# HazyResearch/hyena-dna

Measured on NVIDIA H100. Metric: nucleotides/sec through HyenaOperator fwd+bwd at L=1M d=256, higher is better.
Workload: dtype f32

## Files before the change

hyena-dna_b200/csrc/filter_tc.cuh:

```cuda
#pragma once
#include "fft_passes.cuh"
#include "filter_mlp.cuh"
#include "tc_prims.cuh"

namespace hy {
namespace tc {

constexpr int kTileM = 128;
constexpr uint32_t kSBO = 2048, kLBO = 128;
constexpr int kImgW64 = 64 * 64;
constexpr int kImgW128 = 128 * 64;

__host__ __device__ constexpr uint32_t op_off(int r, int k) {
  return (uint32_t)((r >> 3) * 2048 + (k >> 2) * 128 + (r & 7) * 16 + (k & 3) * 4);
}

constexpr uint32_t kOffAhi = 0, kOffAlo = 32768, kOffW1hi = 65536, kOffW1lo = 81920, kOffW2hi = 98304,
                   kOffW2lo = 114688, kOffW3hi = 131072, kOffW3lo = 163840, kOffMisc = 196608;
constexpr uint32_t kMiscFloats = 64 * 16 + 4 * 64;
constexpr size_t kSmemBytes = kOffMisc + kMiscFloats * 4 + 16;

__host__ __device__ constexpr size_t wimg_floats(int D) { return 4 * (size_t)kImgW64 + (size_t)((D + 127) / 128) * 2 * kImgW128; }

__device__ __noinline__ float sin_ni(float x) { return sinf(x); }
__device__ __noinline__ float cos_ni(float x) { return cosf(x); }

__device__ __forceinline__ void sincos_core(float x, float& sn, float& cs, int& q) {
  const float fq = rintf(x * 0.636619772367581343f);
  q = (int)fq;
  float r = fmaf(fq, -1.5707963705062866f, x);
  r = fmaf(fq, 4.371138828673793e-08f, r);
  r = fmaf(fq, 1.7763568394002505e-15f, r);
  const float s = r * r;
  float ps = fmaf(-1.95152959e-4f, s, 8.33216087e-3f);
  ps = fmaf(ps, s, -1.66666546e-1f);
  sn = fmaf(ps, s * r, r);
  float pc = fmaf(2.44331571e-5f, s, -1.38873163e-3f);
  pc = fmaf(pc, s, 4.16666457e-2f);
  pc = fmaf(pc, s, -0.5f);
  cs = fmaf(pc, s, 1.0f);
}
__device__ __forceinline__ float sin_acc(float x) {
  if (fabsf(x) > 30000.f) return sin_ni(x);
  float sn, cs; int q;
  sincos_core(x, sn, cs, q);
  const float v = (q & 1) ? cs : sn;
  return (q & 2) ? -v : v;
}
__device__ __forceinline__ float cos_acc(float x) {
  if (fabsf(x) > 30000.f) return cos_ni(x);
  float sn, cs; int q;
  sincos_core(x, sn, cs, q);
  const float v = (q & 1) ? sn : cs;
  return ((q + 1) & 2) ? -v : v;
}

struct Frag {
  int r0, t, rh, ch;
  __device__ Frag(int tid) {
    const int warp = tid >> 5, lane = tid & 31, wg = warp >> 2;
    rh = wg & 1; ch = wg >> 1; t = lane & 3;
    r0 = 64 * rh + 16 * (warp & 3) + (lane >> 2);
  }
  __device__ int row(int i) const { return r0 + ((i & 2) ? 8 : 0); }
  __device__ int col(int i, int n_half) const { return ch * n_half + 8 * (i >> 2) + 2 * t + (i & 1); }
};

template <int R>
__device__ __forceinline__ void layer_ss(float (&m)[R], float (&c)[R], uint32_t a_hi, uint32_t a_lo, uint32_t b_hi,
                                         uint32_t b_lo, uint32_t acc0) {
  wgmma_fence();
  fence_regs(m); fence_regs(c);
#pragma unroll
  for (int ks = 0; ks < 8; ++ks)
    wgmma_ss(m, make_desc_ls(a_hi + ks * 2 * kLBO, kLBO, kSBO), make_desc_ls(b_hi + ks * 2 * kLBO, kLBO, kSBO), (acc0 | ks) ? 1u : 0u);
#pragma unroll
  for (int ks = 0; ks < 8; ++ks) {
    wgmma_ss(c, make_desc_ls(a_lo + ks * 2 * kLBO, kLBO, kSBO), make_desc_ls(b_hi + ks * 2 * kLBO, kLBO, kSBO), (acc0 | ks) ? 1u : 0u);
    wgmma_ss(c, make_desc_ls(a_hi + ks * 2 * kLBO, kLBO, kSBO), make_desc_ls(b_lo + ks * 2 * kLBO, kLBO, kSBO), 1u);
  }
  wgmma_commit();
}
template <int R>
__device__ __forceinline__ void layer_wait(float (&m)[R], float (&c)[R]) {
  wgmma_wait<0>();
  fence_regs(m); fence_regs(c);
}

__device__ __forceinline__ void store_pair_split(unsigned char* smem, int r, int k, float x0, float x1) {
  float2 hi, lo;
  split_tf32(x0, hi.x, lo.x);
  split_tf32(x1, hi.y, lo.y);
  const uint32_t off = op_off(r, k);
  *reinterpret_cast<float2*>(smem + kOffAhi + off) = hi;
  *reinterpret_cast<float2*>(smem + kOffAlo + off) = lo;
}
__device__ __forceinline__ void store_frag16(unsigned char* smem, const Frag& f, const float (&a)[16]) {
#pragma unroll
  for (int i = 0; i < 16; i += 2) store_pair_split(smem, f.row(i), f.col(i, 32), a[i], a[i + 1]);
}
__device__ __forceinline__ uint32_t a_rows(uint32_t img, const Frag& f) { return img + (uint32_t)f.rh * 8u * kSBO; }

__global__ void filter_tc_prep_kernel(const float* __restrict__ W1, const float* __restrict__ W2,
                                      const float* __restrict__ W3, int D, float* __restrict__ wimg) {
  const int nh = (D + 127) / 128;
  const int total = 2 * kImgW64 + nh * kImgW128;
  for (int i = blockIdx.x * blockDim.x + threadIdx.x; i < total; i += gridDim.x * blockDim.x) {
    float x;
    float* hi_img;
    float* lo_img;
    int r, k;
    if (i < 2 * kImgW64) {
      const int w = i / kImgW64, e = i % kImgW64;
      r = e / 64; k = e % 64;
      x = (w == 0 ? W1 : W2)[r * 64 + k];
      hi_img = wimg + w * 2 * kImgW64;
      lo_img = hi_img + kImgW64;
    } else {
      const int j = i - 2 * kImgW64, h = j / kImgW128, e = j % kImgW128;
      r = e / 64; k = e % 64;
      const int c = h * 128 + r;
      x = (c < D) ? W3[(size_t)c * 64 + k] : 0.f;
      hi_img = wimg + 4 * kImgW64 + (size_t)h * 2 * kImgW128;
      lo_img = hi_img + kImgW128;
    }
    float hi, lo;
    split_tf32(x, hi, lo);
    hi_img[op_off(r, k) / 4] = hi;
    lo_img[op_off(r, k) / 4] = lo;
  }
}

constexpr int kThreads = 512;

__global__ void __launch_bounds__(kThreads, 1)
filter_tc_fwd_kernel(const FilterParams P, const float* __restrict__ wimg, float* __restrict__ kout, int ntiles) {
  extern __shared__ __align__(1024) unsigned char smem[];
  float* misc = reinterpret_cast<float*>(smem + kOffMisc);
  float* W0s = misc;
  float* b0s = misc + 64 * 16;
  float* b1s = b0s + 64;
  float* b2s = b1s + 64;
  float* frs = b2s + 64;
  const int tid = threadIdx.x;
  const Frag f(tid);
  const uint32_t sbase = smem_u32(smem);
  const int nh = (P.D + 127) / 128;

  for (int i = tid; i < 4 * kImgW64 / 4; i += kThreads)
    cp_async16(smem + kOffW1hi + 16 * i, wimg + 4 * i, true);
  for (int i = tid; i < 64 * 16; i += kThreads) {
    const int r = i / 16, e = i % 16;
    W0s[i] = (e < P.E) ? __ldg(P.W0 + r * P.E + e) : 0.f;
  }
  if (tid < 64) {
    b0s[tid] = __ldg(P.b0 + tid); b1s[tid] = __ldg(P.b1 + tid); b2s[tid] = __ldg(P.b2 + tid);
    frs[tid] = __ldg(P.freq + tid);
  }
  cp_async_wait_all();
  __syncthreads();
  const uint32_t a_hi = a_rows(sbase + kOffAhi, f), a_lo = a_rows(sbase + kOffAlo, f);

  for (int tile = blockIdx.x; tile < ntiles; tile += gridDim.x) {
    const int tb = tile * kTileM;
    {
      const float* src = wimg + 4 * kImgW64;
      for (int i = tid; i < 2 * kImgW128 / 4; i += kThreads) cp_async16(smem + kOffW3hi + 16 * i, src + 4 * i, true);
    }
    {
      float a[16];
#pragma unroll
      for (int h = 0; h < 2; ++h) {
        const int t = tb + f.r0 + 8 * h;
        float z[kMaxE];
#pragma unroll
        for (int e = 0; e < kMaxE; ++e) z[e] = (t < P.L && e < P.E) ? __ldg(P.z + (size_t)t * P.z_stride + e) : 0.f;
#pragma unroll
        for (int i = 0; i < 16; ++i) {
          if (((i >> 1) & 1) != h) continue;
          const int c = f.col(i, 32);
          float acc = b0s[c];
#pragma unroll
          for (int e = 0; e < kMaxE; ++e) acc = fmaf(W0s[c * 16 + e], z[e], acc);
          a[i] = sin_acc(frs[c] * acc);
        }
      }
      store_frag16(smem, f, a);
    }
    fence_async_smem();
    __syncthreads();
#pragma unroll
    for (int layer = 0; layer < 2; ++layer) {
      float m[16], c[16];
      const uint32_t bh = sbase + (layer ? kOffW2hi : kOffW1hi) + (uint32_t)f.ch * 4u * kSBO;
      const uint32_t bl = sbase + (layer ? kOffW2lo : kOffW1lo) + (uint32_t)f.ch * 4u * kSBO;
      layer_ss(m, c, a_hi, a_lo, bh, bl, 0u);
      layer_wait(m, c);
      __syncthreads();
      const float* bs = layer ? b2s : b1s;
      float a[16];
#pragma unroll
      for (int i = 0; i < 16; ++i) {
        const int col = f.col(i, 32);
        a[i] = sin_acc(frs[col] * ((m[i] + c[i]) + bs[col]));
      }
      store_frag16(smem, f, a);
      fence_async_smem();
      __syncthreads();
    }
    float tpos[2];
#pragma unroll
    for (int h = 0; h < 2; ++h) {
      const int t = tb + f.r0 + 8 * h;
      tpos[h] = t < P.L ? __ldg(P.t + t) : 0.f;
    }
    for (int hh = 0; hh < nh; ++hh) {
      cp_async_wait_all();
      fence_async_smem();
      __syncthreads();
      float m[32], c[32];
      layer_ss(m, c, a_hi, a_lo, sbase + kOffW3hi + (uint32_t)f.ch * 8u * kSBO, sbase + kOffW3lo + (uint32_t)f.ch * 8u * kSBO, 0u);
      layer_wait(m, c);
      __syncthreads();
      if (hh + 1 < nh) {
        const float* src = wimg + 4 * kImgW64 + (size_t)(hh + 1) * 2 * kImgW128;
        for (int i = tid; i < 2 * kImgW128 / 4; i += kThreads) cp_async16(smem + kOffW3hi + 16 * i, src + 4 * i, true);
      }
#pragma unroll
      for (int i = 0; i < 32; ++i) {
        const int ch = hh * 128 + f.col(i, 64);
        const int h = (i >> 1) & 1;
        const int t = tb + f.r0 + 8 * h;
        if (ch < P.D && t < P.L) {
          float x = m[i] + c[i];
          if (P.modulate) x *= (expf(-tpos[h] * fabsf(__ldg(P.deltas + ch))) + P.shift);
          kout[(size_t)ch * P.L + t] = x;
        }
      }
    }
  }
}

constexpr int kScratchArrays = 7;

__host__ __device__ constexpr size_t wimg_bwd_floats(int D) {
  return 4 * (size_t)kImgW64 + (size_t)((D + 63) / 64 + 2) * 2 * kImgW64;
}

__global__ void filter_tc_prep_bwd_kernel(const float* __restrict__ W1, const float* __restrict__ W2,
                                          const float* __restrict__ W3, int D, float* __restrict__ wimg) {
  const int nq = (D + 63) / 64;
  const int total = (2 + nq + 2) * kImgW64;
  for (int i = blockIdx.x * blockDim.x + threadIdx.x; i < total; i += gridDim.x * blockDim.x) {
    const int item = i / kImgW64, e = i % kImgW64;
    const int r = e / 64, k = e % 64;
    float x;
    float* hi_img = wimg + (size_t)item * 2 * kImgW64;
    if (item == 0) x = W1[r * 64 + k];
    else if (item == 1) x = W2[r * 64 + k];
    else if (item < 2 + nq) {
      const int c = (item - 2) * 64 + k;
      x = (c < D) ? W3[(size_t)c * 64 + r] : 0.f;
    } else if (item == 2 + nq) x = W2[k * 64 + r];
    else x = W1[k * 64 + r];
    float hi, lo;
    split_tf32(x, hi, lo);
    hi_img[op_off(r, k) / 4] = hi;
    hi_img[kImgW64 + op_off(r, k) / 4] = lo;
  }
}

__device__ __forceinline__ void stream_item(unsigned char* smem, const float* wimg, int item, int tid) {
  const float* src = wimg + (size_t)(2 + item) * 2 * kImgW64;
  unsigned char* dst = smem + kOffW3hi + (item & 1) * 32768;
  for (int i = tid; i < 2 * kImgW64 / 4; i += kThreads) cp_async16(dst + 16 * i, src + 4 * i, true);
}

__device__ __forceinline__ void store_feat16(float* arr, size_t L, const Frag& f, int tb, const float (&a)[16]) {
#pragma unroll
  for (int i = 0; i < 16; ++i) {
    const int t = tb + f.row(i);
    if (t < (int)L) arr[(size_t)f.col(i, 32) * L + t] = a[i];
  }
}

__global__ void __launch_bounds__(kThreads, 1)
filter_tc_bwd_kernel(const FilterParams P, const float* __restrict__ wimg, const float* __restrict__ dk,
                     float* __restrict__ dh, float* __restrict__ scratch, int ntiles) {
  extern __shared__ __align__(1024) unsigned char smem[];
  float* misc = reinterpret_cast<float*>(smem + kOffMisc);
  float* W0s = misc;
  float* b0s = misc + 64 * 16;
  float* b1s = b0s + 64;
  float* b2s = b1s + 64;
  float* frs = b2s + 64;
  const int tid = threadIdx.x;
  const Frag f(tid);
  const uint32_t sbase = smem_u32(smem);
  const int nq = (P.D + 63) / 64;
  const size_t L = (size_t)P.L;
  const size_t arr = L * 64;

  for (int i = tid; i < 4 * kImgW64 / 4; i += kThreads) cp_async16(smem + kOffW1hi + 16 * i, wimg + 4 * i, true);
  for (int i = tid; i < 64 * 16; i += kThreads) {
    const int r = i / 16, e = i % 16;
    W0s[i] = (e < P.E) ? __ldg(P.W0 + r * P.E + e) : 0.f;
  }
  if (tid < 64) {
    b0s[tid] = __ldg(P.b0 + tid); b1s[tid] = __ldg(P.b1 + tid); b2s[tid] = __ldg(P.b2 + tid);
    frs[tid] = __ldg(P.freq + tid);
  }
  cp_async_wait_all();
  __syncthreads();
  const uint32_t a_hi = a_rows(sbase + kOffAhi, f), a_lo = a_rows(sbase + kOffAlo, f);
  const uint32_t bcol = (uint32_t)f.ch * 4u * kSBO;
  float fr[16];
#pragma unroll
  for (int i = 0; i < 16; ++i) fr[i] = frs[f.col(i, 32)];

  for (int tile = blockIdx.x; tile < ntiles; tile += gridDim.x) {
    const int tb = tile * kTileM;
    stream_item(smem, wimg, 0, tid);
    stream_item(smem, wimg, 1, tid);

    float pre1[16], pre2[16], pre3[16], a[16];
#pragma unroll
    for (int h = 0; h < 2; ++h) {
      const int t = tb + f.r0 + 8 * h;
      float z[kMaxE];
#pragma unroll
      for (int e = 0; e < kMaxE; ++e) z[e] = (t < P.L && e < P.E) ? __ldg(P.z + (size_t)t * P.z_stride + e) : 0.f;
#pragma unroll
      for (int i = 0; i < 16; ++i) {
        if (((i >> 1) & 1) != h) continue;
        const int c = f.col(i, 32);
        float acc = b0s[c];
#pragma unroll
        for (int e = 0; e < kMaxE; ++e) acc = fmaf(W0s[c * 16 + e], z[e], acc);
        pre1[i] = acc;
        a[i] = sin_acc(fr[i] * acc);
      }
    }
    store_frag16(smem, f, a);
    store_feat16(scratch + 0 * arr, L, f, tb, a);
    fence_async_smem();
    __syncthreads();
    {
      float m[16], c[16];
      layer_ss(m, c, a_hi, a_lo, sbase + kOffW1hi + bcol, sbase + kOffW1lo + bcol, 0u);
      layer_wait(m, c);
      __syncthreads();
#pragma unroll
      for (int i = 0; i < 16; ++i) { pre2[i] = (m[i] + c[i]) + b1s[f.col(i, 32)]; a[i] = sin_acc(fr[i] * pre2[i]); }
    }
    store_frag16(smem, f, a);
    store_feat16(scratch + 1 * arr, L, f, tb, a);
    fence_async_smem();
    __syncthreads();
    {
      float m[16], c[16];
      layer_ss(m, c, a_hi, a_lo, sbase + kOffW2hi + bcol, sbase + kOffW2lo + bcol, 0u);
      layer_wait(m, c);
      __syncthreads();
#pragma unroll
      for (int i = 0; i < 16; ++i) { pre3[i] = (m[i] + c[i]) + b2s[f.col(i, 32)]; a[i] = sin_acc(fr[i] * pre3[i]); }
    }
    store_feat16(scratch + 2 * arr, L, f, tb, a);

    float tpos[2];
#pragma unroll
    for (int h = 0; h < 2; ++h) {
      const int t = tb + f.r0 + 8 * h;
      tpos[h] = t < P.L ? __ldg(P.t + t) : 0.f;
    }
    float m[16], c[16];
    float nx[16];
#pragma unroll
    for (int i = 0; i < 16; ++i) {
      const int ch = f.col(i, 32), t = tb + f.row(i);
      nx[i] = (ch < P.D && t < P.L) ? __ldg(dk + (size_t)ch * L + t) : 0.f;
    }
    for (int q = 0; q < nq; ++q) {
#pragma unroll
      for (int i = 0; i < 16; ++i) {
        const int ch = q * 64 + f.col(i, 32), t = tb + f.row(i);
        float x = nx[i];
        if (ch < P.D && t < P.L) {
          if (P.modulate) x *= (expf(-tpos[(i >> 1) & 1] * fabsf(__ldg(P.deltas + ch))) + P.shift);
          dh[(size_t)ch * L + t] = x;
        }
        a[i] = x;
      }
      store_frag16(smem, f, a);
      cp_async_wait_all();
      fence_async_smem();
      __syncthreads();
      const uint32_t sb = sbase + kOffW3hi + (q & 1) * 32768;
      layer_ss(m, c, a_hi, a_lo, sb + bcol, sb + 16384u + bcol, q > 0 ? 1u : 0u);
      if (q + 1 < nq) {
#pragma unroll
        for (int i = 0; i < 16; ++i) {
          const int ch = (q + 1) * 64 + f.col(i, 32), t = tb + f.row(i);
          nx[i] = (ch < P.D && t < P.L) ? __ldg(dk + (size_t)ch * L + t) : 0.f;
        }
      }
      layer_wait(m, c);
      __syncthreads();
      stream_item(smem, wimg, q + 2, tid);
    }

    float X[16];
#pragma unroll
    for (int i = 0; i < 16; ++i) {
      const float cs = cos_acc(fr[i] * pre3[i]);
      const float g = (m[i] + c[i]) * cs;
      X[i] = g * pre3[i];
      a[i] = g * fr[i];
    }
    store_feat16(scratch + 5 * arr, L, f, tb, a);
    store_frag16(smem, f, a);
    cp_async_wait_all();
    fence_async_smem();
    __syncthreads();
    {
      const uint32_t sb = sbase + kOffW3hi + (nq & 1) * 32768;
      layer_ss(m, c, a_hi, a_lo, sb + bcol, sb + 16384u + bcol, 0u);
      layer_wait(m, c);
      __syncthreads();
    }
#pragma unroll
    for (int i = 0; i < 16; ++i) {
      const float cs = cos_acc(fr[i] * pre2[i]);
      const float g = (m[i] + c[i]) * cs;
      X[i] = fmaf(g, pre2[i], X[i]);
      a[i] = g * fr[i];
    }
    store_feat16(scratch + 4 * arr, L, f, tb, a);
    store_frag16(smem, f, a);
    fence_async_smem();
    __syncthreads();
    {
      const uint32_t sb = sbase + kOffW3hi + ((nq + 1) & 1) * 32768;
      layer_ss(m, c, a_hi, a_lo, sb + bcol, sb + 16384u + bcol, 0u);
      layer_wait(m, c);
      __syncthreads();
    }
#pragma unroll
    for (int i = 0; i < 16; ++i) {
      const float cs = cos_acc(fr[i] * pre1[i]);
      const float g = (m[i] + c[i]) * cs;
      X[i] = fmaf(g, pre1[i], X[i]);
      a[i] = g * fr[i];
    }
    store_feat16(scratch + 3 * arr, L, f, tb, a);
    store_feat16(scratch + 6 * arr, L, f, tb, X);
  }
}

constexpr int kRedKB = 32;
constexpr int kRedThreads = 512;
constexpr int kRedItems = 12;
constexpr uint32_t kRedSBO = 1024;
__host__ __device__ constexpr uint32_t red_off(int r, int k) {
  return (uint32_t)((r >> 3) * 1024 + (k >> 2) * 128 + (r & 7) * 16 + (k & 3) * 4);
}
constexpr uint32_t kRedImg128 = 128 * kRedKB * 4;
constexpr uint32_t kRedOffDh = 0;
constexpr uint32_t kRedOffAs = 65536;
constexpr uint32_t kRedOffAx = kRedOffAs + 32768;
constexpr uint32_t kRedOffB3 = kRedOffAx + 32768;
constexpr uint32_t kRedOffBs = kRedOffB3 + 16384;
constexpr uint32_t kRedOffBz = kRedOffBs + 36864;
constexpr uint32_t kRedOffMisc = kRedOffBz + 4096;
constexpr size_t kRedSmemBytes = kRedOffMisc + 64;

template <int R>
__device__ __forceinline__ void issue_red(float (&d)[R], uint32_t a_hi, uint32_t a_lo, uint32_t b_hi, uint32_t b_lo, uint32_t first_acc) {
  uint32_t acc = first_acc;
#pragma unroll
  for (int pass = 0; pass < 3; ++pass) {
    const uint32_t a = (pass == 1) ? a_lo : a_hi;
    const uint32_t b = (pass == 2) ? b_lo : b_hi;
#pragma unroll
    for (int ks = 0; ks < kRedKB / 8; ++ks) {
      wgmma_ss(d, make_desc_ls(a + ks * 2 * kLBO, kLBO, kRedSBO), make_desc_ls(b + ks * 2 * kLBO, kLBO, kRedSBO), acc);
      acc = 1;
    }
  }
}

__device__ __forceinline__ float4 load4_row(const float* __restrict__ src, size_t t, size_t L, bool v4) {
  float4 x = make_float4(0.f, 0.f, 0.f, 0.f);
  if (v4 && t + 3 < L) return __ldg(reinterpret_cast<const float4*>(src + t));
  if (t < L) x.x = __ldg(src + t);
  if (t + 1 < L) x.y = __ldg(src + t + 1);
  if (t + 2 < L) x.z = __ldg(src + t + 2);
  if (t + 3 < L) x.w = __ldg(src + t + 3);
  return x;
}

struct RedArgs {
  const float* dh;
  const float* scratch;
  const float* zT;
  float* dW0; float* db0; float* dW1; float* db1; float* dW2; float* db2; float* dW3; float* dfreq;
  int L, D, E;
};

struct RedItem { const float* src; uint32_t off; uint32_t lo_off; };
__device__ __forceinline__ RedItem red_item(const RedArgs& R, int it, int tid) {
  const size_t L = (size_t)R.L;
  const int nrow = R.D + 7 * 64 + R.E;
  const int pc = (tid >> 3) & 7;
  const int row = (((tid + kRedThreads * it) >> 6) << 3) + (tid & 7);
  RedItem m{nullptr, 0u, 0u};
  uint32_t img = 0, lo = 0;
  int r = 0;
  if (row < R.D) {
    m.src = R.dh + (size_t)row * L; img = kRedOffDh + (row >> 7) * 32768; lo = 16384; r = row & 127;
  } else if (row < nrow) {
    const int q = row - R.D;
    if (q < 7 * 64) {
      const int arr = q >> 6, f = q & 63;
      m.src = R.scratch + ((size_t)arr * 64 + f) * L;
      switch (arr) {
        case 0: img = kRedOffBs; lo = 18432; r = 64 + f; break;
        case 1: img = kRedOffBs; lo = 18432; r = f; break;
        case 2: img = kRedOffB3; lo = 8192; r = f; break;
        case 3: img = kRedOffAx; lo = 16384; r = f; break;
        case 4: img = kRedOffAs; lo = 16384; r = 64 + f; break;
        case 5: img = kRedOffAs; lo = 16384; r = f; break;
        default: img = kRedOffAx; lo = 16384; r = 64 + f; break;
      }
    } else {
      const int e = q - 7 * 64;
      m.src = R.zT + (size_t)e * L; img = kRedOffBz; lo = 2048; r = e;
    }
  }
  m.off = img + red_off(r, 4 * pc);
  m.lo_off = lo;
  return m;
}

constexpr int kRedChain = 8;

__device__ __forceinline__ void red_flush(const RedArgs& R, const Frag& f, int nmt, const float (&g1)[2][16],
                                          const float (&g2)[36], const float (&g3)[4]) {
  for (int mt = 0; mt < nmt; ++mt) {
#pragma unroll
    for (int i = 0; i < 16; ++i) {
      const int c = mt * 128 + f.row(i);
      if (c < R.D) atomicAdd(R.dW3 + (size_t)c * 64 + f.col(i, 32), g1[mt][i]);
    }
  }
#pragma unroll
  for (int i = 0; i < 36; ++i) {
    const int r = f.row(i), n = f.col(i, 72);
    if (n == 128) atomicAdd(((r < 64) ? R.db2 : R.db1) + (r & 63), g2[i]);
    else if (r < 64 && n < 64) atomicAdd(R.dW2 + r * 64 + n, g2[i]);
    else if (r >= 64 && n >= 64 && n < 128) atomicAdd(R.dW1 + (r - 64) * 64 + (n - 64), g2[i]);
  }
#pragma unroll
  for (int i = 0; i < 4; ++i) {
    const int r = f.row(i), n = f.col(i, 8);
    if (r < 64) {
      if (n < R.E) atomicAdd(R.dW0 + r * R.E + n, g3[i]);
      else if (n == 8) atomicAdd(R.db0 + r, g3[i]);
    } else if (n == 8) {
      atomicAdd(R.dfreq + (r - 64), g3[i]);
    }
  }
}

__global__ void __launch_bounds__(kRedThreads, 1) filter_tc_red_kernel(const RedArgs R, int nblocks) {
  extern __shared__ __align__(1024) unsigned char smem[];
  const int tid = threadIdx.x;
  const Frag f(tid);
  const uint32_t sbase = smem_u32(smem);
  const int nmt = (R.D + 127) / 128;
  const size_t L = (size_t)R.L;
  const bool v4 = (R.L & 3) == 0;
  const int pc = (tid >> 3) & 7;

  for (uint32_t i = tid; i < kRedOffMisc / 16; i += kRedThreads) reinterpret_cast<float4*>(smem)[i] = make_float4(0.f, 0.f, 0.f, 0.f);
  __syncthreads();
  for (int i = tid; i < 16 * kRedKB; i += kRedThreads) {
    const int r = 128 + i / kRedKB, k = i % kRedKB;
    *reinterpret_cast<float*>(smem + kRedOffBs + red_off(r, k)) = 1.f;
  }
  for (int i = tid; i < 8 * kRedKB; i += kRedThreads) {
    const int r = 8 + i / kRedKB, k = i % kRedKB;
    *reinterpret_cast<float*>(smem + kRedOffBz + red_off(r, k)) = 1.f;
  }
  __syncthreads();

  float g1[2][16], g2[36], g3[4];
  const uint32_t arow = (uint32_t)f.rh * 8u * kRedSBO;
  bool first = true;
  int chain = 0;
  for (int blk = blockIdx.x; blk < nblocks; blk += gridDim.x) {
    const size_t t = (size_t)blk * kRedKB + 4 * pc;
    if (!first) {
      wgmma_wait<0>();
      fence_regs(g1[0]); fence_regs(g1[1]); fence_regs(g2); fence_regs(g3);
      __syncthreads();
    }
#pragma unroll
    for (int half = 0; half < 2; ++half) {
      constexpr int kH = kRedItems / 2;
      float4 x[kH];
      RedItem m[kH];
#pragma unroll
      for (int j = 0; j < kH; ++j) {
        m[j] = red_item(R, half * kH + j, tid);
        x[j] = m[j].src ? load4_row(m[j].src, t, L, v4) : make_float4(0.f, 0.f, 0.f, 0.f);
      }
#pragma unroll
      for (int j = 0; j < kH; ++j) {
        if (m[j].src) {
          float4 hi, lo;
          split_tf32(x[j].x, hi.x, lo.x); split_tf32(x[j].y, hi.y, lo.y);
          split_tf32(x[j].z, hi.z, lo.z); split_tf32(x[j].w, hi.w, lo.w);
          *reinterpret_cast<float4*>(smem + m[j].off) = hi;
          *reinterpret_cast<float4*>(smem + m[j].off + m[j].lo_off) = lo;
        }
      }
    }
    fence_async_smem();
    __syncthreads();
    const uint32_t acc0 = chain ? 1u : 0u;
    wgmma_fence();
    fence_regs(g1[0]); fence_regs(g1[1]); fence_regs(g2); fence_regs(g3);
#pragma unroll
    for (int mt = 0; mt < 2; ++mt)
      if (mt < nmt)
        issue_red(g1[mt], sbase + kRedOffDh + mt * 32768 + arow, sbase + kRedOffDh + mt * 32768 + 16384 + arow,
                  sbase + kRedOffB3 + f.ch * 4 * kRedSBO, sbase + kRedOffB3 + 8192 + f.ch * 4 * kRedSBO, acc0);
    issue_red(g2, sbase + kRedOffAs + arow, sbase + kRedOffAs + 16384 + arow, sbase + kRedOffBs + f.ch * 9 * kRedSBO,
              sbase + kRedOffBs + 18432 + f.ch * 9 * kRedSBO, acc0);
    issue_red(g3, sbase + kRedOffAx + arow, sbase + kRedOffAx + 16384 + arow, sbase + kRedOffBz + f.ch * kRedSBO,
              sbase + kRedOffBz + 2048 + f.ch * kRedSBO, acc0);
    wgmma_commit();
    first = false;
    if (++chain == kRedChain) {
      wgmma_wait<0>();
      fence_regs(g1[0]); fence_regs(g1[1]); fence_regs(g2); fence_regs(g3);
      red_flush(R, f, nmt, g1, g2, g3);
      chain = 0;
    }
  }
  if (chain == 0) return;
  wgmma_wait<0>();
  fence_regs(g1[0]); fence_regs(g1[1]); fence_regs(g2); fence_regs(g3);
  red_flush(R, f, nmt, g1, g2, g3);
}

}
}
```

hyena-dna_b200/csrc/tc_prims.cuh:

```cuda
#pragma once
#include <cuda_runtime.h>
#include <stdint.h>

namespace hy {
namespace tc {

__device__ __forceinline__ float to_tf32(float x) {
  return __uint_as_float((__float_as_uint(x) + 0x1000u) & 0xFFFFE000u);
}
__device__ __forceinline__ void split_tf32(float x, float& hi, float& lo) {
  hi = to_tf32(x);
  lo = to_tf32(x - hi);
}

__device__ __forceinline__ uint32_t smem_u32(const void* p) { return (uint32_t)__cvta_generic_to_shared(p); }

__device__ __forceinline__ uint64_t make_desc_ls(uint32_t saddr, uint32_t lbo, uint32_t sbo) {
  uint64_t d = 0;
  d |= (uint64_t)((saddr & 0x3FFFFu) >> 4);
  d |= (uint64_t)(lbo >> 4) << 16;
  d |= (uint64_t)(sbo >> 4) << 32;
  return d;
}

__device__ __forceinline__ void wgmma_fence() { asm volatile("wgmma.fence.sync.aligned;" ::: "memory"); }
__device__ __forceinline__ void wgmma_commit() { asm volatile("wgmma.commit_group.sync.aligned;" ::: "memory"); }
template <int N>
__device__ __forceinline__ void wgmma_wait() { asm volatile("wgmma.wait_group.sync.aligned %0;" ::"n"(N) : "memory"); }
template <int R>
__device__ __forceinline__ void fence_regs(float (&d)[R]) {
#pragma unroll
  for (int i = 0; i < R; ++i) asm volatile("" : "+f"(d[i])::"memory");
}

template <int R, int C>
__device__ __forceinline__ void fence_frags(uint32_t (&a)[R][C]) {
#pragma unroll
  for (int i = 0; i < R; ++i)
#pragma unroll
    for (int j = 0; j < C; ++j) asm volatile("" : "+r"(a[i][j])::"memory");
}

template <int R>
__device__ __forceinline__ void setmaxnreg_inc() { asm volatile("setmaxnreg.inc.sync.aligned.u32 %0;" ::"n"(R)); }
template <int R>
__device__ __forceinline__ void setmaxnreg_dec() { asm volatile("setmaxnreg.dec.sync.aligned.u32 %0;" ::"n"(R)); }

__device__ __forceinline__ void wgmma_ss_n8(float (&d)[4], uint64_t da, uint64_t db, uint32_t scale_d) {
  asm volatile(
      "{\n\t.reg .pred p;\n\tsetp.ne.b32 p, %6, 0;\n\t"
      "wgmma.mma_async.sync.aligned.m64n8k8.f32.tf32.tf32 "
      "{%0, %1, %2, %3}, %4, %5, p, 1, 1;\n\t}\n"
      : "+f"(d[0]), "+f"(d[1]), "+f"(d[2]), "+f"(d[3])
      : "l"(da), "l"(db), "r"(scale_d));
}
__device__ __forceinline__ void wgmma_ss_n32(float (&d)[16], uint64_t da, uint64_t db, uint32_t scale_d) {
  asm volatile(
      "{\n\t.reg .pred p;\n\tsetp.ne.b32 p, %18, 0;\n\t"
      "wgmma.mma_async.sync.aligned.m64n32k8.f32.tf32.tf32 "
      "{%0, %1, %2, %3, %4, %5, %6, %7, %8, %9, %10, %11, %12, %13, %14, %15}, %16, %17, p, 1, 1;\n\t}\n"
      : "+f"(d[0]), "+f"(d[1]), "+f"(d[2]), "+f"(d[3]), "+f"(d[4]), "+f"(d[5]), "+f"(d[6]), "+f"(d[7]), "+f"(d[8]), "+f"(d[9]), "+f"(d[10]), "+f"(d[11]), "+f"(d[12]), "+f"(d[13]), "+f"(d[14]), "+f"(d[15])
      : "l"(da), "l"(db), "r"(scale_d));
}
__device__ __forceinline__ void wgmma_ss_n64(float (&d)[32], uint64_t da, uint64_t db, uint32_t scale_d) {
  asm volatile(
      "{\n\t.reg .pred p;\n\tsetp.ne.b32 p, %34, 0;\n\t"
      "wgmma.mma_async.sync.aligned.m64n64k8.f32.tf32.tf32 "
      "{%0, %1, %2, %3, %4, %5, %6, %7, %8, %9, %10, %11, %12, %13, %14, %15, %16, %17, %18, %19, %20, %21, %22, %23, %24, %25, %26, %27, %28, %29, %30, %31}, %32, %33, p, 1, 1;\n\t}\n"
      : "+f"(d[0]), "+f"(d[1]), "+f"(d[2]), "+f"(d[3]), "+f"(d[4]), "+f"(d[5]), "+f"(d[6]), "+f"(d[7]), "+f"(d[8]), "+f"(d[9]), "+f"(d[10]), "+f"(d[11]), "+f"(d[12]), "+f"(d[13]), "+f"(d[14]), "+f"(d[15]), "+f"(d[16]), "+f"(d[17]), "+f"(d[18]), "+f"(d[19]), "+f"(d[20]), "+f"(d[21]), "+f"(d[22]), "+f"(d[23]), "+f"(d[24]), "+f"(d[25]), "+f"(d[26]), "+f"(d[27]), "+f"(d[28]), "+f"(d[29]), "+f"(d[30]), "+f"(d[31])
      : "l"(da), "l"(db), "r"(scale_d));
}
__device__ __forceinline__ void wgmma_ss_n72(float (&d)[36], uint64_t da, uint64_t db, uint32_t scale_d) {
  asm volatile(
      "{\n\t.reg .pred p;\n\tsetp.ne.b32 p, %38, 0;\n\t"
      "wgmma.mma_async.sync.aligned.m64n72k8.f32.tf32.tf32 "
      "{%0, %1, %2, %3, %4, %5, %6, %7, %8, %9, %10, %11, %12, %13, %14, %15, %16, %17, %18, %19, %20, %21, %22, %23, %24, %25, %26, %27, %28, %29, %30, %31, %32, %33, %34, %35}, %36, %37, p, 1, 1;\n\t}\n"
      : "+f"(d[0]), "+f"(d[1]), "+f"(d[2]), "+f"(d[3]), "+f"(d[4]), "+f"(d[5]), "+f"(d[6]), "+f"(d[7]), "+f"(d[8]), "+f"(d[9]), "+f"(d[10]), "+f"(d[11]), "+f"(d[12]), "+f"(d[13]), "+f"(d[14]), "+f"(d[15]), "+f"(d[16]), "+f"(d[17]), "+f"(d[18]), "+f"(d[19]), "+f"(d[20]), "+f"(d[21]), "+f"(d[22]), "+f"(d[23]), "+f"(d[24]), "+f"(d[25]), "+f"(d[26]), "+f"(d[27]), "+f"(d[28]), "+f"(d[29]), "+f"(d[30]), "+f"(d[31]), "+f"(d[32]), "+f"(d[33]), "+f"(d[34]), "+f"(d[35])
      : "l"(da), "l"(db), "r"(scale_d));
}
__device__ __forceinline__ void wgmma_rs_n128(float (&d)[64], const uint32_t (&a)[4], uint64_t db, uint32_t scale_d) {
  asm volatile(
      "{\n\t.reg .pred p;\n\tsetp.ne.b32 p, %69, 0;\n\t"
      "wgmma.mma_async.sync.aligned.m64n128k8.f32.tf32.tf32 "
      "{%0, %1, %2, %3, %4, %5, %6, %7, %8, %9, %10, %11, %12, %13, %14, %15, %16, %17, %18, %19, %20, %21, %22, %23, %24, %25, %26, %27, %28, %29, %30, %31, %32, %33, %34, %35, %36, %37, %38, %39, %40, %41, %42, %43, %44, %45, %46, %47, %48, %49, %50, %51, %52, %53, %54, %55, %56, %57, %58, %59, %60, %61, %62, %63}, {%64, %65, %66, %67}, %68, p, 1, 1;\n\t}\n"
      : "+f"(d[0]), "+f"(d[1]), "+f"(d[2]), "+f"(d[3]), "+f"(d[4]), "+f"(d[5]), "+f"(d[6]), "+f"(d[7]), "+f"(d[8]), "+f"(d[9]), "+f"(d[10]), "+f"(d[11]), "+f"(d[12]), "+f"(d[13]), "+f"(d[14]), "+f"(d[15]), "+f"(d[16]), "+f"(d[17]), "+f"(d[18]), "+f"(d[19]), "+f"(d[20]), "+f"(d[21]), "+f"(d[22]), "+f"(d[23]), "+f"(d[24]), "+f"(d[25]), "+f"(d[26]), "+f"(d[27]), "+f"(d[28]), "+f"(d[29]), "+f"(d[30]), "+f"(d[31]), "+f"(d[32]), "+f"(d[33]), "+f"(d[34]), "+f"(d[35]), "+f"(d[36]), "+f"(d[37]), "+f"(d[38]), "+f"(d[39]), "+f"(d[40]), "+f"(d[41]), "+f"(d[42]), "+f"(d[43]), "+f"(d[44]), "+f"(d[45]), "+f"(d[46]), "+f"(d[47]), "+f"(d[48]), "+f"(d[49]), "+f"(d[50]), "+f"(d[51]), "+f"(d[52]), "+f"(d[53]), "+f"(d[54]), "+f"(d[55]), "+f"(d[56]), "+f"(d[57]), "+f"(d[58]), "+f"(d[59]), "+f"(d[60]), "+f"(d[61]), "+f"(d[62]), "+f"(d[63])
      : "r"(a[0]), "r"(a[1]), "r"(a[2]), "r"(a[3]), "l"(db), "r"(scale_d));
}

__device__ __forceinline__ void wgmma_ss(float (&d)[4], uint64_t da, uint64_t db, uint32_t sc) { wgmma_ss_n8(d, da, db, sc); }
__device__ __forceinline__ void wgmma_ss(float (&d)[16], uint64_t da, uint64_t db, uint32_t sc) { wgmma_ss_n32(d, da, db, sc); }
__device__ __forceinline__ void wgmma_ss(float (&d)[32], uint64_t da, uint64_t db, uint32_t sc) { wgmma_ss_n64(d, da, db, sc); }
__device__ __forceinline__ void wgmma_ss(float (&d)[36], uint64_t da, uint64_t db, uint32_t sc) { wgmma_ss_n72(d, da, db, sc); }

__device__ __forceinline__ void mbar_init(uint32_t mbar, uint32_t count) {
  asm volatile("mbarrier.init.shared::cta.b64 [%0], %1;" ::"r"(mbar), "r"(count) : "memory");
  asm volatile("fence.mbarrier_init.release.cluster;" ::: "memory");
}
__device__ __forceinline__ void fence_async_smem() { asm volatile("fence.proxy.async.shared::cta;" ::: "memory"); }

__device__ __forceinline__ void mbar_arrive(uint32_t mbar) {
  asm volatile("mbarrier.arrive.shared::cta.b64 _, [%0];" ::"r"(mbar) : "memory");
}
__device__ __forceinline__ void mbar_arrive_after_loads(uint32_t mbar, uint32_t dep, uint32_t zero) {
  const uint32_t cnt = 1u + (dep & zero);
  asm volatile("mbarrier.arrive.shared::cta.b64 _, [%0], %1;" ::"r"(mbar), "r"(cnt) : "memory");
}
__device__ __forceinline__ void mbar_arrive_expect_tx(uint32_t mbar, uint32_t bytes) {
  asm volatile("mbarrier.arrive.expect_tx.shared::cta.b64 _, [%0], %1;" ::"r"(mbar), "r"(bytes) : "memory");
}
__device__ __forceinline__ void bulk_g2s(uint32_t smem_dst, const void* gsrc, uint32_t bytes, uint32_t mbar) {
  asm volatile("cp.async.bulk.shared::cluster.global.mbarrier::complete_tx::bytes [%0], [%1], %2, [%3];"
               ::"r"(smem_dst), "l"(gsrc), "r"(bytes), "r"(mbar)
               : "memory");
}
__device__ __forceinline__ void tma_load_2d(uint32_t smem_dst, const void* tmap, int c0, int c1, uint32_t mbar) {
  asm volatile("cp.async.bulk.tensor.2d.shared::cluster.global.mbarrier::complete_tx::bytes [%0], [%1, {%3, %4}], [%2];"
               ::"r"(smem_dst), "l"(tmap), "r"(mbar), "r"(c0), "r"(c1)
               : "memory");
}
__device__ __forceinline__ void tma_load_3d(uint32_t smem_dst, const void* tmap, int c0, int c1, int c2, uint32_t mbar) {
  asm volatile("cp.async.bulk.tensor.3d.shared::cluster.global.mbarrier::complete_tx::bytes [%0], [%1, {%3, %4, %5}], [%2];"
               ::"r"(smem_dst), "l"(tmap), "r"(mbar), "r"(c0), "r"(c1), "r"(c2)
               : "memory");
}
__device__ __forceinline__ void tma_prefetch_desc(const void* tmap) {
  asm volatile("prefetch.tensormap [%0];" ::"l"(tmap) : "memory");
}

__device__ __forceinline__ void mbar_wait_u(uint32_t mbar, uint32_t parity) {
  uint32_t done = 0;
  const long long t0 = clock64();
  while (!done) {
    asm volatile(
        "{\n\t.reg .pred p;\n\t"
        "mbarrier.try_wait.parity.shared::cta.b64 p, [%1], %2;\n\t"
        "selp.u32 %0, 1, 0, p;\n\t}\n"
        : "=r"(done)
        : "r"(mbar), "r"(parity)
        : "memory");
    if (!done && clock64() - t0 > 4000000000LL) __trap();
  }
}

}
}
```

Before: 18.79 million.

## Recompute layer-0 preactivations and add L2 prefetch in reduction loop

Factors the first-layer positional MLP into a helper with a runtime loop over E, and in the backward filter kernel recomputes the layer-0 preactivations at the end instead of keeping pre1 live across the whole tile. The per-thread frequency array is replaced with shared-memory lookups, all to cut register pressure in a 512-thread, one-block-per-SM kernel. Separately, the reduction kernel issues L2 prefetches for the next block's source rows after committing the wgmma group. The trade-off is extra global z loads, FMAs and shared loads, plus prefetch instructions in the loop.

```diff
diff --git a/hyena-dna_b200/csrc/filter_tc.cuh b/hyena-dna_b200/csrc/filter_tc.cuh
--- a/hyena-dna_b200/csrc/filter_tc.cuh
+++ b/hyena-dna_b200/csrc/filter_tc.cuh
@@ -131,6 +131,26 @@
   }
 }
 
+__device__ __forceinline__ void layer0_pre(const FilterParams& P, const float* W0s, const float* b0s, const Frag& f, int tb,
+                                           float (&pre)[16]) {
+#pragma unroll
+  for (int i = 0; i < 16; ++i) pre[i] = b0s[f.col(i, 32)];
+#pragma unroll
+  for (int h = 0; h < 2; ++h) {
+    const int t = tb + f.r0 + 8 * h;
+    const float* zr = P.z + (size_t)t * P.z_stride;
+#pragma unroll 1
+    for (int e = 0; e < P.E; ++e) {
+      const float z = t < P.L ? __ldg(zr + e) : 0.f;
+#pragma unroll
+      for (int i = 0; i < 16; ++i)
+        if (((i >> 1) & 1) == h) pre[i] = fmaf(W0s[f.col(i, 32) * 16 + e], z, pre[i]);
+    }
+  }
+#pragma unroll
+  for (int i = 0; i < 16; ++i) pre[i] += 0.f;
+}
+
 constexpr int kThreads = 512;
 
 __global__ void __launch_bounds__(kThreads, 1)
@@ -169,22 +189,9 @@
     }
     {
       float a[16];
-#pragma unroll
-      for (int h = 0; h < 2; ++h) {
-        const int t = tb + f.r0 + 8 * h;
-        float z[kMaxE];
-#pragma unroll
-        for (int e = 0; e < kMaxE; ++e) z[e] = (t < P.L && e < P.E) ? __ldg(P.z + (size_t)t * P.z_stride + e) : 0.f;
-#pragma unroll
-        for (int i = 0; i < 16; ++i) {
-          if (((i >> 1) & 1) != h) continue;
-          const int c = f.col(i, 32);
-          float acc = b0s[c];
-#pragma unroll
-          for (int e = 0; e < kMaxE; ++e) acc = fmaf(W0s[c * 16 + e], z[e], acc);
-          a[i] = sin_acc(frs[c] * acc);
-        }
-      }
+      layer0_pre(P, W0s, b0s, f, tb, a);
+#pragma unroll
+      for (int i = 0; i < 16; ++i) a[i] = sin_acc(frs[f.col(i, 32)] * a[i]);
       store_frag16(smem, f, a);
     }
     fence_async_smem();
@@ -314,33 +321,17 @@
   __syncthreads();
   const uint32_t a_hi = a_rows(sbase + kOffAhi, f), a_lo = a_rows(sbase + kOffAlo, f);
   const uint32_t bcol = (uint32_t)f.ch * 4u * kSBO;
-  float fr[16];
-#pragma unroll
-  for (int i = 0; i < 16; ++i) fr[i] = frs[f.col(i, 32)];
+  const auto fr = [&](int i) { return frs[f.col(i, 32)]; };
 
   for (int tile = blockIdx.x; tile < ntiles; tile += gridDim.x) {
     const int tb = tile * kTileM;
     stream_item(smem, wimg, 0, tid);
     stream_item(smem, wimg, 1, tid);
 
-    float pre1[16], pre2[16], pre3[16], a[16];
-#pragma unroll
-    for (int h = 0; h < 2; ++h) {
-      const int t = tb + f.r0 + 8 * h;
-      float z[kMaxE];
-#pragma unroll
-      for (int e = 0; e < kMaxE; ++e) z[e] = (t < P.L && e < P.E) ? __ldg(P.z + (size_t)t * P.z_stride + e) : 0.f;
-#pragma unroll
-      for (int i = 0; i < 16; ++i) {
-        if (((i >> 1) & 1) != h) continue;
-        const int c = f.col(i, 32);
-        float acc = b0s[c];
-#pragma unroll
-        for (int e = 0; e < kMaxE; ++e) acc = fmaf(W0s[c * 16 + e], z[e], acc);
-        pre1[i] = acc;
-        a[i] = sin_acc(fr[i] * acc);
-      }
-    }
+    float pre2[16], pre3[16], a[16];
+    layer0_pre(P, W0s, b0s, f, tb, a);
+#pragma unroll
+    for (int i = 0; i < 16; ++i) a[i] = sin_acc(fr(i) * a[i]);
     store_frag16(smem, f, a);
     store_feat16(scratch + 0 * arr, L, f, tb, a);
     fence_async_smem();
@@ -351,7 +342,7 @@
       layer_wait(m, c);
       __syncthreads();
 #pragma unroll
-      for (int i = 0; i < 16; ++i) { pre2[i] = (m[i] + c[i]) + b1s[f.col(i, 32)]; a[i] = sin_acc(fr[i] * pre2[i]); }
+      for (int i = 0; i < 16; ++i) { pre2[i] = (m[i] + c[i]) + b1s[f.col(i, 32)]; a[i] = sin_acc(fr(i) * pre2[i]); }
     }
     store_frag16(smem, f, a);
     store_feat16(scratch + 1 * arr, L, f, tb, a);
@@ -363,7 +354,7 @@
       layer_wait(m, c);
       __syncthreads();
 #pragma unroll
-      for (int i = 0; i < 16; ++i) { pre3[i] = (m[i] + c[i]) + b2s[f.col(i, 32)]; a[i] = sin_acc(fr[i] * pre3[i]); }
+      for (int i = 0; i < 16; ++i) { pre3[i] = (m[i] + c[i]) + b2s[f.col(i, 32)]; a[i] = sin_acc(fr(i) * pre3[i]); }
     }
     store_feat16(scratch + 2 * arr, L, f, tb, a);
 
@@ -412,10 +403,10 @@
     float X[16];
 #pragma unroll
     for (int i = 0; i < 16; ++i) {
-      const float cs = cos_acc(fr[i] * pre3[i]);
+      const float cs = cos_acc(fr(i) * pre3[i]);
       const float g = (m[i] + c[i]) * cs;
       X[i] = g * pre3[i];
-      a[i] = g * fr[i];
+      a[i] = g * fr(i);
     }
     store_feat16(scratch + 5 * arr, L, f, tb, a);
     store_frag16(smem, f, a);
@@ -430,10 +421,10 @@
     }
 #pragma unroll
     for (int i = 0; i < 16; ++i) {
-      const float cs = cos_acc(fr[i] * pre2[i]);
+      const float cs = cos_acc(fr(i) * pre2[i]);
       const float g = (m[i] + c[i]) * cs;
       X[i] = fmaf(g, pre2[i], X[i]);
-      a[i] = g * fr[i];
+      a[i] = g * fr(i);
     }
     store_feat16(scratch + 4 * arr, L, f, tb, a);
     store_frag16(smem, f, a);
@@ -445,12 +436,14 @@
       layer_wait(m, c);
       __syncthreads();
     }
+    float pre1[16];
+    layer0_pre(P, W0s, b0s, f, tb, pre1);
 #pragma unroll
     for (int i = 0; i < 16; ++i) {
-      const float cs = cos_acc(fr[i] * pre1[i]);
+      const float cs = cos_acc(fr(i) * pre1[i]);
       const float g = (m[i] + c[i]) * cs;
       X[i] = fmaf(g, pre1[i], X[i]);
-      a[i] = g * fr[i];
+      a[i] = g * fr(i);
     }
     store_feat16(scratch + 3 * arr, L, f, tb, a);
     store_feat16(scratch + 6 * arr, L, f, tb, X);
@@ -642,6 +635,14 @@
               sbase + kRedOffBz + 2048 + f.ch * kRedSBO, acc0);
     wgmma_commit();
     first = false;
+    if (blk + (int)gridDim.x < nblocks) {
+      const size_t tn = (size_t)(blk + gridDim.x) * kRedKB + 4 * pc;
+#pragma unroll 1
+      for (int it = 0; it < kRedItems; ++it) {
+        const RedItem m = red_item(R, it, tid);
+        if (m.src && tn < L) prefetch_l2(m.src + tn);
+      }
+    }
     if (++chain == kRedChain) {
       wgmma_wait<0>();
       fence_regs(g1[0]); fence_regs(g1[1]); fence_regs(g2); fence_regs(g3);
diff --git a/hyena-dna_b200/csrc/tc_prims.cuh b/hyena-dna_b200/csrc/tc_prims.cuh
--- a/hyena-dna_b200/csrc/tc_prims.cuh
+++ b/hyena-dna_b200/csrc/tc_prims.cuh
@@ -123,6 +123,7 @@
                ::"r"(smem_dst), "l"(tmap), "r"(mbar), "r"(c0), "r"(c1), "r"(c2)
                : "memory");
 }
+__device__ __forceinline__ void prefetch_l2(const void* p) { asm volatile("prefetch.global.L2 [%0];" ::"l"(p)); }
 __device__ __forceinline__ void tma_prefetch_desc(const void* tmap) {
   asm volatile("prefetch.tensormap [%0];" ::"l"(tmap) : "memory");
 }
```

Result: faster. 20.32 million (median of 6 runs) (+8.1%).
